# daigo0927/tf-raft

Measured on AMD Instinct MI355X. Metric: image-pairs/sec at 448×512 iters_pred=24; final-iter EPE vs TF ref, higher is better.
Workload: dtype f32; 1 GPU; RAFT forward BASELINE configs[1]: batch 4/GPU 448x512 iters_pred=24 random weights; pairs_per_gpu=4, global_batch=4, parallelism=dp1, collective=none

## Files before the change

tf_raft_amd/csrc/conv_wino4.h:

```cpp
#pragma once
#include "conv_mfma.h"

typedef float f32x2 __attribute__((ext_vector_type(2)));
typedef unsigned int u32x2 __attribute__((ext_vector_type(2)));

#include <type_traits>
#include <utility>

#ifdef RAFT_WINO4_SCALAR
struct alignas(8) w4v2 {
    float x, y;
    __device__ __forceinline__ float operator[](int i) const { return i ? y : x; }
};
__device__ __forceinline__ w4v2 operator+(w4v2 a, w4v2 b) { return {a.x + b.x, a.y + b.y}; }
__device__ __forceinline__ w4v2 operator-(w4v2 a, w4v2 b) { return {a.x - b.x, a.y - b.y}; }
__device__ __forceinline__ w4v2 operator*(float k, w4v2 a) { return {k * a.x, k * a.y}; }
#else
typedef f32x2 w4v2;
#endif

template <class F, int... I>
__device__ __forceinline__ void w4_static_for_impl(F &f, std::integer_sequence<int, I...>) {
    (f(std::integral_constant<int, I>{}), ...);
}
template <int N, class F>
__device__ __forceinline__ void w4_static_for(F &&f) {
    w4_static_for_impl(f, std::make_integer_sequence<int, N>{});
}
#define W4_TAPS(X)                                                                                                       \
    X(0) X(1) X(2) X(3) X(4) X(5) X(6) X(7) X(8) X(9) X(10) X(11) X(12) X(13) X(14) X(15) X(16) X(17) X(18) X(19) X(20) X(21)   \
    X(22) X(23) X(24) X(25) X(26) X(27) X(28) X(29) X(30) X(31) X(32) X(33) X(34) X(35)

#ifndef RAFT_WINO4_PF
#define RAFT_WINO4_PF 7
#endif
#ifdef RAFT_WINO4_NOSB
#define W4_SB()
#else
#define W4_SB() __builtin_amdgcn_sched_barrier(0)
#endif
#ifdef RAFT_WINO4_NOSNOP
#define W4_PAD ""
#else
#define W4_PAD "s_nop 1\n\t"
#endif
#define W4_MFMA4                                                                                                          \
    W4_PAD "v_mfma_f32_16x16x4_f32 %0, %2, %4, %0\n\tv_mfma_f32_16x16x4_f32 %1, %2, %6, %1\n\t"                          \
           "v_mfma_f32_16x16x4_f32 %0, %3, %5, %0\n\tv_mfma_f32_16x16x4_f32 %1, %3, %7, %1"
#ifndef RAFT_WINO4_ATAPS
#define RAFT_WINO4_ATAPS 31
#endif
#ifndef RAFT_WINO4_ABL
#define RAFT_WINO4_ABL 0
#endif

namespace wino4 {
constexpr float PA = 0.625f, PB = 1.5f;
constexpr float A2 = PA * PA, B2 = PB * PB, SS = A2 + B2, PP = A2 * B2, A3 = A2 * PA, B3 = B2 * PB;
constexpr int TW = 64, HWP = TW + 2;
constexpr int RS = 1124;
constexpr int NTHR = 256;
constexpr int PF = RAFT_WINO4_PF, NR = 8;
constexpr int W4_ATAPS = RAFT_WINO4_ATAPS;
#ifndef RAFT_WINO4_LAG
#define RAFT_WINO4_LAG 12
#endif
constexpr int LOAD_SLOT0 = 0, STORE_LAG = RAFT_WINO4_LAG;
static_assert(PF >= 1 && PF < NR, "prefetch distance must fit the fragment ring");
__device__ __forceinline__ constexpr int tap_row(int ph, int row) { return ph == 0 ? 1 + row : (ph == 1 ? 3 + row : 5 * row); }
}

#pragma clang diagnostic push
#pragma clang diagnostic ignored "-Wunused-lambda-capture"
template <int EPI, int KS = 1, int PRE = 0, int STATS = 0>
__global__ void __launch_bounds__(256, 1) conv_wino4_kernel(ConvArgs p) {
    using namespace wino4;
    static_assert(EPI == EPI_LINEAR || EPI == EPI_RELU || EPI == EPI_RES, "winograd F(4x4) kernel: linear / relu / residual epilogues");
    static_assert(KS == 1 || KS == 2, "K split: 1 or 2");
    static_assert((!PRE && !STATS) || KS == 1, "encoder variants: two row blocks per workgroup");
    constexpr int TH = KS == 1 ? 8 : 4, HH = TH + 2, HP = HH * HWP;
    constexpr int A_BUF = HH * RS + 16;
    constexpr int NA = (HP * 4 * KS + NTHR - 1) / NTHR;
    static_assert(LOAD_SLOT0 + NA - 1 + STORE_LAG < 60, "halo writes must precede the chunk's barrier (slot 60)");
    __shared__ __attribute__((aligned(16))) float smem[2 * KS * A_BUF];

    const int tid = threadIdx.x, lane = tid & 63;
    const int w = __builtin_amdgcn_readfirstlane(tid >> 6);
    const int G = lane >> 4, LR = lane & 15;
    const int rb = KS == 1 ? (w & 1) : 0, cbp = KS == 1 ? (w >> 1) : (w & 1), ks = KS == 1 ? 0 : (w >> 1);
    const int tiles_x = (p.W + TW - 1) / TW, tiles_y = (p.H + TH - 1) / TH;
    const int ntn = p.npad / 64;
    const int M = p.B * p.H * p.W;

    int bid = blockIdx.x;
    {
        const int nwg = gridDim.x, xcd = bid & 7, q = nwg >> 3, r = nwg & 7;
        bid = (xcd < r ? xcd * (q + 1) : r * (q + 1) + (xcd - r) * q) + (bid >> 3);
    }
    int mt = bid / ntn, nt = bid - mt * ntn;
#ifdef RAFT_WINO4_XCD
    {
        const int nwg = gridDim.x, xcd = blockIdx.x & 7, idx = blockIdx.x >> 3;
        if ((nwg & 7) == 0 && (ntn & 7) == 0) {
            const int per = ntn >> 3;
            nt = xcd + 8 * (idx % per);
            mt = idx / per;
        } else if ((nwg & 7) == 0 && 8 % ntn == 0) {
            const int g = 8 / ntn;
            nt = xcd % ntn;
            mt = idx * g + xcd / ntn;
        }
    }
#endif
    const int tx0 = mt % tiles_x, ty0 = (mt / tiles_x) % tiles_y, b = mt / (tiles_x * tiles_y);
    const int y0 = ty0 * TH, x0 = tx0 * TW;
    const int n0 = nt * 64;
    const int cin = p.c0 + p.c1;
    const int nch = cin >> 4;
    const int nst = nch / KS;

    const __amdgpu_buffer_rsrc_t rs0 = __builtin_amdgcn_make_buffer_rsrc(
        (void *)p.a0, 0, (int)((((long)M - 1) * p.lda0 + p.c0) * 4), 0x00020000);
    const __amdgpu_buffer_rsrc_t rsw = __builtin_amdgcn_make_buffer_rsrc(
        (void *)p.wp, 0, (int)((long)36 * cin * p.npad * 4), 0x00020000);

    unsigned pixoff[NA];
    int lds_off[NA], pixi[NA];
    unsigned okbits = 0;
#pragma unroll
    for (int i = 0; i < NA; ++i) {
        const int item = tid + NTHR * i;
        const int hq = item >> 2, c4 = item & 3;
        const int s2 = hq / HP, hp = hq - s2 * HP;
        const int hy = hp / HWP, hx = hp - hy * HWP;
        const int yy = y0 - 1 + hy, xx = x0 - 1 + hx;
        const bool ok = (s2 < KS) & ((unsigned)yy < (unsigned)p.H) & ((unsigned)xx < (unsigned)p.W);
        pixi[i] = ok ? (b * p.H + yy) * p.W + xx : -1;
        okbits |= ok ? 1u << i : 0u;
        pixoff[i] = ok ? (unsigned)((pixi[i] * p.lda0 + s2 * 16 + c4 * 4) * 4) : RAFT_OOB;
        lds_off[i] = s2 < KS ? s2 * A_BUF + hy * RS + hx * 16 + (hx >> 2) * 4 + 2 * c4 : HH * RS;
    }
    f32x4 ra[NA];
    f32x2 pre_sc[2], pre_sh[2];
    __amdgpu_buffer_rsrc_t rsn = rs0;
    int soff_n = 0;
    bool on_first = true;
    auto next_source = [&](int st) {
        const int ch = st * 16 * KS;
        const bool first = ch < p.c0, live = st < nst && !(RAFT_WINO4_ABL & 4);
        const float *base = first ? p.a0 : (p.c1 ? p.a1 : p.a0);
        const int ext = first ? (int)((((long)M - 1) * p.lda0 + p.c0) * 4) : (p.c1 ? (int)((((long)M - 1) * p.lda1 + p.c1) * 4) : 0);
        rsn = __builtin_amdgcn_make_buffer_rsrc((void *)base, 0, live ? ext : 0, 0x00020000);
        soff_n = (first ? ch : ch - p.c0) * 4;
        if constexpr (PRE) {
            const int cq = (st < nst ? ch : 0) + (tid & 3) * 4;
            const f32x4 sc = *(const f32x4 *)(p.pre_scale + (long)b * cin + cq), sh = *(const f32x4 *)(p.pre_shift + (long)b * cin + cq);
            pre_sc[0] = f32x2{sc[0], sc[1]};
            pre_sc[1] = f32x2{sc[2], sc[3]};
            pre_sh[0] = f32x2{sh[0], sh[1]};
            pre_sh[1] = f32x2{sh[2], sh[3]};
            return;
        }
        if (on_first && !first) {
            on_first = false;
#pragma unroll
            for (int i = 0; i < NA; ++i)
                pixoff[i] = pixi[i] >= 0 ? (unsigned)((pixi[i] * p.lda1 + (((tid + NTHR * i) >> 2) / HP) * 16 + (tid & 3) * 4) * 4) : RAFT_OOB;
        }
    };
    auto gload_item = [&](int i) {
        ra[i] = __builtin_bit_cast(f32x4, __builtin_amdgcn_raw_buffer_load_b128(rsn, (int)pixoff[i], soff_n, 0));
    };
    auto lstore_item = [&](int i, int buf) {
        float *dst = smem + buf * (KS * A_BUF) + lds_off[i];
        f32x2 lo = f32x2{ra[i][0], ra[i][1]}, hi = f32x2{ra[i][2], ra[i][3]};
        if constexpr (PRE) {
            const bool ok = (okbits >> i) & 1u;
            const f32x2 zero = f32x2{0.f, 0.f};
            lo = __builtin_elementwise_max(__builtin_elementwise_fma(lo, pre_sc[0], pre_sh[0]), zero);
            hi = __builtin_elementwise_max(__builtin_elementwise_fma(hi, pre_sc[1], pre_sh[1]), zero);
            lo = ok ? lo : zero;
            hi = ok ? hi : zero;
        }
        *(f32x2 *)dst = lo;
        *(f32x2 *)(dst + 8) = hi;
    };

    const int a_lane = ks * A_BUF + (4 * rb) * RS + 68 * LR + 2 * G;
    auto rd = [&](int buf, int r, int j, int h) -> w4v2 {
        return *(const w4v2 *)(smem + a_lane + (buf * (KS * A_BUF) + r * RS + 16 * j + 4 * (j >> 2) + 8 * h));
    };
    const unsigned b_lane = (unsigned)(((G * (p.npad >> 5) + (n0 >> 5) + cbp) * 16 + LR) * 16);
    const unsigned qstride = (unsigned)(4 * p.npad) * 8u;
    unsigned wrow = (unsigned)ks * 72u * qstride;
    f32x4 fb[NR];
    auto frag_b = [&](int q, bool skip = false) {
        if (KS == 2 && skip) wrow += 72u * qstride;
        fb[q & (NR - 1)] = __builtin_bit_cast(f32x4, __builtin_amdgcn_raw_buffer_load_b128(rsw, (int)b_lane, (int)wrow, 0));
        wrow += qstride;
        asm volatile("" : "+s"(wrow));
    };

#define X(t) f32x4 accA_##t = f32x4{0.f, 0.f, 0.f, 0.f}, accB_##t = f32x4{0.f, 0.f, 0.f, 0.f};
    W4_TAPS(X)
#undef X
    int acc_end_ = 0;
#define X(t) &accA_##t, &accB_##t,
    auto mma4 = [W4_TAPS(X) & acc_end_](auto tap, float a0, float a1, f32x4 bw) {
#undef X
        constexpr int T = decltype(tap)::value;
#define X(t)                                                                                                                 \
    if constexpr (T == t) {                                                                                                 \
        if constexpr (t < W4_ATAPS)                                                                                         \
            asm volatile(W4_MFMA4 : "+a"(accA_##t), "+a"(accB_##t) : "v"(a0), "v"(a1), "v"(bw[0]), "v"(bw[1]), "v"(bw[2]), "v"(bw[3])); \
        else                                                                                                                \
            asm volatile(W4_MFMA4 : "+v"(accA_##t), "+v"(accB_##t) : "v"(a0), "v"(a1), "v"(bw[0]), "v"(bw[1]), "v"(bw[2]), "v"(bw[3])); \
    }
        W4_TAPS(X)
#undef X
    };
#define X(t) &accA_##t, &accB_##t,
    auto acc_of = [W4_TAPS(X) & acc_end_](auto tile) -> f32x4 {
#undef X
        constexpr int IDX = decltype(tile)::value;
#define X(t)                                       \
    if constexpr (IDX == 2 * t) return accA_##t;   \
    if constexpr (IDX == 2 * t + 1) return accB_##t;
        W4_TAPS(X)
#undef X
    };

    w4v2 R[4][6], W[2][2][6], e0, e5;
    auto s1_pair = [&](int par, int ph, int j) {
        if (RAFT_WINO4_ABL & 2) {
            W[par][0][j] = W[par][1][j] = w4v2{1.f, 1.f};
            return;
        }
        const float c2 = ph == 0 ? B2 : A2, c1 = ph == 0 ? PA : PB;
        const w4v2 t1 = R[3][j] - c2 * R[1][j], t2 = R[2][j] - c2 * R[0][j];
        W[par][0][j] = t1 + c1 * t2;
        W[par][1][j] = t1 - c1 * t2;
    };
    auto s1_edge = [&](int par, int j) {
        if (RAFT_WINO4_ABL & 2) {
            W[par][0][j] = W[par][1][j] = w4v2{1.f, 1.f};
            return;
        }
        W[par][0][j] = (R[3][j] - SS * R[1][j]) + PP * e0;
        W[par][1][j] = (e5 - SS * R[2][j]) + PP * R[0][j];
    };
    w4v2 V[6];
    auto s2_calc = [&](const w4v2 *wr, int tx) {
        if (RAFT_WINO4_ABL & 16) {
            V[tx] = wr[tx];
            return;
        }
        if (tx == 0) {
            V[0] = (wr[4] - SS * wr[2]) + PP * wr[0];
        } else if (tx == 1) {
            const w4v2 t1 = wr[4] - B2 * wr[2], t2 = wr[3] - B2 * wr[1];
            V[1] = t1 + PA * t2;
            V[2] = t1 - PA * t2;
        } else if (tx == 3) {
            const w4v2 t1 = wr[4] - A2 * wr[2], t2 = wr[3] - A2 * wr[1];
            V[3] = t1 + PB * t2;
            V[4] = t1 - PB * t2;
        } else if (tx == 5) {
            V[5] = (wr[5] - SS * wr[3]) + PP * wr[1];
        }
    };

    next_source(0);
#pragma unroll
    for (int i = 0; i < NA; ++i) gload_item(i);
#pragma unroll
    for (int q = 0; q < PF; ++q) frag_b(q);
#pragma unroll
    for (int i = 0; i < NA; ++i) lstore_item(i, 0);
    raft_barrier_lds();
#pragma unroll
    for (int j = 0; j < 6; ++j) {
#pragma unroll
        for (int r = 0; r < 4; ++r) R[r][j] = (RAFT_WINO4_ABL & 2) ? w4v2{1.f, 1.f} : rd(0, r + 1, j, 0);
        s1_pair(0, 0, j);
    }
    s2_calc(W[0][0], 0);

    auto chunk = [&](auto buf_c, int c) {
        constexpr int BUF = decltype(buf_c)::value;
        next_source(c + 1);
        w4_static_for<6>([&](auto inst_c) {
            constexpr int inst = decltype(inst_c)::value;
            constexpr int h = inst / 3, ph = inst % 3, par = inst & 1;
            constexpr int n_h = ph == 2 ? 1 - h : h;
            constexpr int n_buf = (ph == 2 && h == 1) ? 1 - BUF : BUF;
            if (inst == 5) raft_barrier_lds();
            w4_static_for<12>([&](auto u_c) {
                constexpr int u = decltype(u_c)::value;
                constexpr int row = u / 6, tx = u % 6, j = u >> 1;
                constexpr int q = inst * 12 + u;
                constexpr int t = tap_row(ph, row) * 6 + tx;
                if (!(RAFT_WINO4_ABL & 1)) frag_b((q + PF) % 72, q + PF == 72);
                if (!(RAFT_WINO4_ABL & 2)) {
                    if constexpr (ph == 1 && (u & 1) == 0) {
                        e0 = rd(BUF, 0, j, h);
                        e5 = rd(BUF, 5, j, h);
                    }
                    if constexpr (ph == 2 && (u & 1) == 0) {
#pragma unroll
                        for (int r = 0; r < 4; ++r) R[r][j] = rd(n_buf, r + 1, j, n_h);
                    }
                }
                if constexpr ((u & 1) == 1) {
                    if constexpr (ph == 0) s1_pair(par ^ 1, 1, j);
                    if constexpr (ph == 1) s1_edge(par ^ 1, j);
                    if constexpr (ph == 2) s1_pair(par ^ 1, 0, j);
                }
                {
                    constexpr int li = q - LOAD_SLOT0, si = q - LOAD_SLOT0 - STORE_LAG;
                    if constexpr (li >= 0 && li < NA) gload_item(li);
                    if constexpr (si >= 0 && si < NA) lstore_item(si, 1 - BUF);
                }
                W4_SB();
                mma4(std::integral_constant<int, t>{}, V[tx][0], V[tx][1], fb[q & (NR - 1)]);
                W4_SB();
                if constexpr (u < 11) s2_calc(W[par][(u + 1) / 6], (u + 1) % 6);
                if constexpr (u == 11) s2_calc(W[par ^ 1][0], 0);
            });
        });
    };
    for (int st = 0; st < nst; st += 2) {
        chunk(std::integral_constant<int, 0>{}, st);
        chunk(std::integral_constant<int, 1>{}, st + 1);
    }

    asm volatile("s_nop 15\n\ts_nop 15" ::: "memory");
    __builtin_amdgcn_sched_barrier(0);

    constexpr bool HAS_E0 = EPI == EPI_RES;
    const __amdgpu_buffer_rsrc_t ro0 = __builtin_amdgcn_make_buffer_rsrc(
        (void *)p.o0, 0, (int)((((long)M - 1) * p.ldo0 + p.nvalid) * 4), 0x00020000);
    const __amdgpu_buffer_rsrc_t re0 = __builtin_amdgcn_make_buffer_rsrc(
        (void *)(HAS_E0 ? (const void *)p.e0 : (const void *)p.o0), 0,
        HAS_E0 ? (int)((((long)M - 1) * p.lde0 + p.nvalid) * 4) : 0, 0x00020000);
    auto bstore = [](float v, __amdgpu_buffer_rsrc_t r, unsigned voff, int soff) {
        __builtin_amdgcn_raw_buffer_store_b32(__builtin_bit_cast(unsigned, v), r, (int)voff, soff, 0);
    };
    auto bload = [](__amdgpu_buffer_rsrc_t r, unsigned voff, int soff) {
        return __builtin_bit_cast(float, __builtin_amdgcn_raw_buffer_load_b32(r, (int)voff, soff, 0));
    };
    const bool interior = (y0 + TH <= p.H) & (x0 + TW <= p.W);
    int tid_e = threadIdx.x;
    asm volatile("" : "+v"(tid_e));
    const int G_e = (tid_e >> 4) & 3, LR_e = tid_e & 15, rb_e = (tid_e >> 6) & 1, cbp_e = tid_e >> 7;
    const int xb = x0 + 16 * G_e;
    const int ks_e = KS == 1 ? 0 : (tid_e >> 7), cb_e = KS == 1 ? cbp_e : ((tid_e >> 6) & 1), w_e = tid_e >> 6;
    constexpr int NROW = KS == 1 ? 4 : 2;
    unsigned bo[NROW], be[NROW];
    bool rowok[NROW];
#pragma unroll
    for (int i = 0; i < NROW; ++i) {
        const int yy = y0 + (KS == 1 ? 4 * rb_e : 2 * ks_e) + i;
        const unsigned pix0 = (unsigned)((b * p.H + yy) * p.W + xb);
        bo[i] = pix0 * p.ldo0 * 4u;
        be[i] = HAS_E0 ? pix0 * p.lde0 * 4u : 0u;
        rowok[i] = yy < p.H;
    }
    float bias2[2];
    unsigned nofs[2];
    bool nok2[2];
#pragma unroll
    for (int j = 0; j < 2; ++j) {
        const int n = n0 + (cb_e * 2 + j) * 16 + LR_e;
        nok2[j] = n < p.nvalid;
        nofs[j] = (unsigned)n * 4u;
        bias2[j] = p.bias[n];
    }
    float st1[2] = {0.f, 0.f}, st2[2] = {0.f, 0.f};
    auto emit = [&](int j, int i, int rh, const f32x2 *Y) {
        const float bias = bias2[j];
        const unsigned vo = nok2[j] ? bo[i] + nofs[j] : RAFT_OOB, ve = (HAS_E0 && nok2[j]) ? be[i] + nofs[j] : RAFT_OOB;
#pragma unroll
        for (int rr = 0; rr < 2; ++rr) {
            const int r = 2 * rh + rr;
            float xv[4];
            if (HAS_E0) {
#pragma unroll
                for (int jx = 0; jx < 4; ++jx) {
                    const unsigned dead = (interior | (rowok[i] & (xb + 4 * r + jx < p.W))) ? 0u : RAFT_OOB;
                    xv[jx] = bload(re0, ve | dead, (4 * r + jx) * p.lde0 * 4);
                }
            }
#pragma unroll
            for (int jx = 0; jx < 4; ++jx) {
                float v = Y[jx][rr] + bias;
                if (EPI == EPI_RES) {
                    v = fmaxf(xv[jx] + fmaxf(v, 0.f), 0.f);
                } else {
                    if (EPI == EPI_RELU) v = fmaxf(v, 0.f);
                    v *= p.scale;
                }
                if ((RAFT_WINO4_ABL & 8) && v != 12345.678f) continue;
                const unsigned dead = (interior | (rowok[i] & (xb + 4 * r + jx < p.W))) ? 0u : RAFT_OOB;
                if constexpr (STATS) {
                    unsigned dd = dead;
                    asm volatile("" : "+v"(dd));
                    const float vs = __builtin_bit_cast(float, __builtin_bit_cast(unsigned, v) & ~(unsigned)((int)dd >> 31));
                    st1[j] += vs;
                    st2[j] = fmaf(vs, vs, st2[j]);
                }
                bstore(v, ro0, vo | dead, (4 * r + jx) * p.ldo0 * 4);
            }
        }
    };
    f32x2 *xch = (f32x2 *)smem;
    if (KS == 2) raft_barrier_lds();
    w4_static_for<4>([&](auto jr_c) {
        constexpr int j = decltype(jr_c)::value >> 1, rh = decltype(jr_c)::value & 1;
        f32x2 T[4][6], keep[2][4];
        w4_static_for<6>([&](auto tx_c) {
            constexpr int tx = decltype(tx_c)::value;
            auto half = [&](f32x4 a) { return f32x2{a[2 * rh], a[2 * rh + 1]}; };
            const f32x2 m0 = half(acc_of(std::integral_constant<int, 2 * tx + j>{})),
                        m1 = half(acc_of(std::integral_constant<int, 2 * (6 + tx) + j>{})),
                        m2 = half(acc_of(std::integral_constant<int, 2 * (12 + tx) + j>{})),
                        m3 = half(acc_of(std::integral_constant<int, 2 * (18 + tx) + j>{})),
                        m4 = half(acc_of(std::integral_constant<int, 2 * (24 + tx) + j>{})),
                        m5 = half(acc_of(std::integral_constant<int, 2 * (30 + tx) + j>{}));
            const f32x2 sa = m1 + m2, da = m1 - m2, sb = m3 + m4, db = m3 - m4;
            T[0][tx] = m0 + (sa + sb);
            T[1][tx] = PA * da + PB * db;
            T[2][tx] = A2 * sa + B2 * sb;
            T[3][tx] = (A3 * da + B3 * db) + m5;
            __builtin_amdgcn_sched_barrier(0);
        });
#pragma unroll
        for (int i = 0; i < 4; ++i) {
            const f32x2 sa = T[i][1] + T[i][2], da = T[i][1] - T[i][2], sb = T[i][3] + T[i][4], db = T[i][3] - T[i][4];
            f32x2 Y[4];
            Y[0] = T[i][0] + (sa + sb);
            Y[1] = PA * da + PB * db;
            Y[2] = A2 * sa + B2 * sb;
            Y[3] = (A3 * da + B3 * db) + T[i][5];
            if (KS == 1) {
                emit(j, i, rh, Y);
            } else {
                const bool mine = (i >> 1) == ks_e;
#pragma unroll
                for (int jx = 0; jx < 4; ++jx) {
                    if (mine)
                        keep[i & 1][jx] = Y[jx];
                    else
                        xch[(((((j * 2 + rh) * 4 + (w_e ^ 2)) * 2 + (i & 1)) * 4 + jx) << 6) + (tid_e & 63)] = Y[jx];
                }
            }
            __builtin_amdgcn_sched_barrier(0);
        }
        if (KS == 2) {
            raft_barrier_lds();
#pragma unroll
            for (int i2 = 0; i2 < 2; ++i2) {
                f32x2 Y[4];
#pragma unroll
                for (int jx = 0; jx < 4; ++jx)
                    Y[jx] = keep[i2][jx] + xch[(((((j * 2 + rh) * 4 + w_e) * 2 + i2) * 4 + jx) << 6) + (tid_e & 63)];
                emit(j, i2, rh, Y);
            }
        }
    });
    if constexpr (STATS) {
#pragma unroll
        for (int j = 0; j < 2; ++j) {
            float s1 = st1[j], s2 = st2[j];
            s1 += __shfl_xor(s1, 16, 64);
            s2 += __shfl_xor(s2, 16, 64);
            s1 += __shfl_xor(s1, 32, 64);
            s2 += __shfl_xor(s2, 32, 64);
            const int n = n0 + (cb_e * 2 + j) * 16 + LR_e;
            if (G_e == 0) *(float2 *)(p.stats + ((long)(2 * mt + rb_e) * p.npad + n) * 2) = make_float2(s1, s2);
        }
    }
}

#pragma clang diagnostic pop
```

Baseline: 388.2 image-pairs/s.

## Split Winograd tap rows across waves with doubled column tiles and LDS accumulator exchange

Reorganizes the Winograd F(4x4) conv kernel so each wave handles half of the transform tap rows (chosen by th) for all 64 output columns, instead of all taps for a 32-column half. Each A fragment now feeds eight MFMAs across two B fragments, which halves redundant input-transform work per wave. After the main loop, the waves swap their partial accumulators through LDS so each ends up with complete tiles for the epilogue. Prefetch distance, store lag and the AGPR split are retuned to fit the shorter 36-slot loop, at the cost of an extra LDS exchange, two barriers and larger shared memory.

```diff
diff --git a/tf_raft_amd/csrc/conv_wino4.h b/tf_raft_amd/csrc/conv_wino4.h
--- a/tf_raft_amd/csrc/conv_wino4.h
+++ b/tf_raft_amd/csrc/conv_wino4.h
@@ -27,12 +27,10 @@
 __device__ __forceinline__ void w4_static_for(F &&f) {
     w4_static_for_impl(f, std::make_integer_sequence<int, N>{});
 }
-#define W4_TAPS(X)                                                                                                       \
-    X(0) X(1) X(2) X(3) X(4) X(5) X(6) X(7) X(8) X(9) X(10) X(11) X(12) X(13) X(14) X(15) X(16) X(17) X(18) X(19) X(20) X(21)   \
-    X(22) X(23) X(24) X(25) X(26) X(27) X(28) X(29) X(30) X(31) X(32) X(33) X(34) X(35)
+#define W4_LT(X) X(0) X(1) X(2) X(3) X(4) X(5) X(6) X(7) X(8) X(9) X(10) X(11) X(12) X(13) X(14) X(15) X(16) X(17)
 
 #ifndef RAFT_WINO4_PF
-#define RAFT_WINO4_PF 7
+#define RAFT_WINO4_PF 4
 #endif
 #ifdef RAFT_WINO4_NOSB
 #define W4_SB()
@@ -44,11 +42,13 @@
 #else
 #define W4_PAD "s_nop 1\n\t"
 #endif
-#define W4_MFMA4                                                                                                          \
-    W4_PAD "v_mfma_f32_16x16x4_f32 %0, %2, %4, %0\n\tv_mfma_f32_16x16x4_f32 %1, %2, %6, %1\n\t"                          \
-           "v_mfma_f32_16x16x4_f32 %0, %3, %5, %0\n\tv_mfma_f32_16x16x4_f32 %1, %3, %7, %1"
-#ifndef RAFT_WINO4_ATAPS
-#define RAFT_WINO4_ATAPS 31
+#define W4_MFMA8                                                                                                          \
+    W4_PAD "v_mfma_f32_16x16x4_f32 %0, %4, %6, %0\n\tv_mfma_f32_16x16x4_f32 %1, %4, %8, %1\n\t"                          \
+           "v_mfma_f32_16x16x4_f32 %2, %4, %10, %2\n\tv_mfma_f32_16x16x4_f32 %3, %4, %12, %3\n\t"                        \
+           "v_mfma_f32_16x16x4_f32 %0, %5, %7, %0\n\tv_mfma_f32_16x16x4_f32 %1, %5, %9, %1\n\t"                          \
+           "v_mfma_f32_16x16x4_f32 %2, %5, %11, %2\n\tv_mfma_f32_16x16x4_f32 %3, %5, %13, %3"
+#ifndef RAFT_WINO4_ATILES
+#define RAFT_WINO4_ATILES 62
 #endif
 #ifndef RAFT_WINO4_ABL
 #define RAFT_WINO4_ABL 0
@@ -61,13 +61,13 @@
 constexpr int RS = 1124;
 constexpr int NTHR = 256;
 constexpr int PF = RAFT_WINO4_PF, NR = 8;
-constexpr int W4_ATAPS = RAFT_WINO4_ATAPS;
+constexpr int W4_ATILES = RAFT_WINO4_ATILES;
+static_assert(W4_ATILES % 2 == 0 && W4_ATILES <= 64, "AGPR tiles: pairs of column blocks, at most 256 registers");
 #ifndef RAFT_WINO4_LAG
-#define RAFT_WINO4_LAG 12
+#define RAFT_WINO4_LAG 6
 #endif
 constexpr int LOAD_SLOT0 = 0, STORE_LAG = RAFT_WINO4_LAG;
 static_assert(PF >= 1 && PF < NR, "prefetch distance must fit the fragment ring");
-__device__ __forceinline__ constexpr int tap_row(int ph, int row) { return ph == 0 ? 1 + row : (ph == 1 ? 3 + row : 5 * row); }
 }
 
 #pragma clang diagnostic push
@@ -81,13 +81,14 @@
     constexpr int TH = KS == 1 ? 8 : 4, HH = TH + 2, HP = HH * HWP;
     constexpr int A_BUF = HH * RS + 16;
     constexpr int NA = (HP * 4 * KS + NTHR - 1) / NTHR;
-    static_assert(LOAD_SLOT0 + NA - 1 + STORE_LAG < 60, "halo writes must precede the chunk's barrier (slot 60)");
-    __shared__ __attribute__((aligned(16))) float smem[2 * KS * A_BUF];
+    static_assert(LOAD_SLOT0 + NA - 1 + STORE_LAG < 30, "halo writes must precede the chunk's barrier (slot 30)");
+    constexpr int XS = 4 * 36 * 64 * 4;
+    __shared__ __attribute__((aligned(16))) float smem[2 * KS * A_BUF > XS ? 2 * KS * A_BUF : XS];
 
     const int tid = threadIdx.x, lane = tid & 63;
     const int w = __builtin_amdgcn_readfirstlane(tid >> 6);
     const int G = lane >> 4, LR = lane & 15;
-    const int rb = KS == 1 ? (w & 1) : 0, cbp = KS == 1 ? (w >> 1) : (w & 1), ks = KS == 1 ? 0 : (w >> 1);
+    const int rb = KS == 1 ? (w & 1) : 0, th = KS == 1 ? (w >> 1) : (w & 1), ks = KS == 1 ? 0 : (w >> 1);
     const int tiles_x = (p.W + TW - 1) / TW, tiles_y = (p.H + TH - 1) / TH;
     const int ntn = p.npad / 64;
     const int M = p.B * p.H * p.W;
@@ -187,67 +188,84 @@
     };
 
     const int a_lane = ks * A_BUF + (4 * rb) * RS + 68 * LR + 2 * G;
+    const int e_lane = a_lane + th * RS;
     auto rd = [&](int buf, int r, int j, int h) -> w4v2 {
         return *(const w4v2 *)(smem + a_lane + (buf * (KS * A_BUF) + r * RS + 16 * j + 4 * (j >> 2) + 8 * h));
     };
-    const unsigned b_lane = (unsigned)(((G * (p.npad >> 5) + (n0 >> 5) + cbp) * 16 + LR) * 16);
+    auto rd_e = [&](int buf, int r, int j, int h) -> w4v2 {
+        return *(const w4v2 *)(smem + e_lane + (buf * (KS * A_BUF) + r * RS + 16 * j + 4 * (j >> 2) + 8 * h));
+    };
+    const unsigned b_lane = (unsigned)(((G * (p.npad >> 5) + (n0 >> 5)) * 16 + LR) * 16);
     const unsigned qstride = (unsigned)(4 * p.npad) * 8u;
-    unsigned wrow = (unsigned)ks * 72u * qstride;
-    f32x4 fb[NR];
-    auto frag_b = [&](int q, bool skip = false) {
-        if (KS == 2 && skip) wrow += 72u * qstride;
-        fb[q & (NR - 1)] = __builtin_bit_cast(f32x4, __builtin_amdgcn_raw_buffer_load_b128(rsw, (int)b_lane, (int)wrow, 0));
+    const unsigned skip_pe = (unsigned)(12 - 6 * th) * qstride;
+    const unsigned skip_ep = (unsigned)(6 + 6 * th) * qstride;
+    unsigned wrow = ((unsigned)ks * 72u + 12u * (unsigned)th) * qstride;
+    f32x4 fb[NR][2];
+    auto frag_b = [&](int pos, int ring, bool first = false) {
+        if (!first && pos % 18 == 12) wrow += skip_pe;
+        if (!first && pos % 18 == 0) wrow += skip_ep + (KS == 2 && pos == 0 ? 72u * qstride : 0u);
+        fb[ring][0] = __builtin_bit_cast(f32x4, __builtin_amdgcn_raw_buffer_load_b128(rsw, (int)b_lane, (int)wrow, 0));
+        fb[ring][1] = __builtin_bit_cast(f32x4, __builtin_amdgcn_raw_buffer_load_b128(rsw, (int)(b_lane + 256u), (int)wrow, 0));
         wrow += qstride;
         asm volatile("" : "+s"(wrow));
     };
 
-#define X(t) f32x4 accA_##t = f32x4{0.f, 0.f, 0.f, 0.f}, accB_##t = f32x4{0.f, 0.f, 0.f, 0.f};
-    W4_TAPS(X)
+#define X(s) f32x4 acc0_##s = f32x4{0.f, 0.f, 0.f, 0.f}, acc1_##s = f32x4{0.f, 0.f, 0.f, 0.f}, \
+                   acc2_##s = f32x4{0.f, 0.f, 0.f, 0.f}, acc3_##s = f32x4{0.f, 0.f, 0.f, 0.f};
+    W4_LT(X)
 #undef X
     int acc_end_ = 0;
-#define X(t) &accA_##t, &accB_##t,
-    auto mma4 = [W4_TAPS(X) & acc_end_](auto tap, float a0, float a1, f32x4 bw) {
-#undef X
-        constexpr int T = decltype(tap)::value;
-#define X(t)                                                                                                                 \
-    if constexpr (T == t) {                                                                                                 \
-        if constexpr (t < W4_ATAPS)                                                                                         \
-            asm volatile(W4_MFMA4 : "+a"(accA_##t), "+a"(accB_##t) : "v"(a0), "v"(a1), "v"(bw[0]), "v"(bw[1]), "v"(bw[2]), "v"(bw[3])); \
+#define X(s) &acc0_##s, &acc1_##s, &acc2_##s, &acc3_##s,
+    auto mma8 = [W4_LT(X) & acc_end_](auto tap, float a0, float a1, f32x4 b0, f32x4 b1) {
+#undef X
+        constexpr int S = decltype(tap)::value;
+#define W4_OPS(C0, C1, C2, C3, s)                                                                                            \
+    : C0(acc0_##s), C1(acc1_##s), C2(acc2_##s), C3(acc3_##s)                                                                  \
+    : "v"(a0), "v"(a1), "v"(b0[0]), "v"(b0[1]), "v"(b0[2]), "v"(b0[3]), "v"(b1[0]), "v"(b1[1]), "v"(b1[2]), "v"(b1[3])
+#define X(s)                                                                                                                 \
+    if constexpr (S == s) {                                                                                                 \
+        if constexpr (4 * s + 4 <= W4_ATILES)                                                                               \
+            asm volatile(W4_MFMA8 W4_OPS("+a", "+a", "+a", "+a", s));                                                       \
+        else if constexpr (4 * s + 2 <= W4_ATILES)                                                                          \
+            asm volatile(W4_MFMA8 W4_OPS("+a", "+a", "+v", "+v", s));                                                       \
         else                                                                                                                \
-            asm volatile(W4_MFMA4 : "+v"(accA_##t), "+v"(accB_##t) : "v"(a0), "v"(a1), "v"(bw[0]), "v"(bw[1]), "v"(bw[2]), "v"(bw[3])); \
-    }
-        W4_TAPS(X)
-#undef X
-    };
-#define X(t) &accA_##t, &accB_##t,
-    auto acc_of = [W4_TAPS(X) & acc_end_](auto tile) -> f32x4 {
-#undef X
-        constexpr int IDX = decltype(tile)::value;
-#define X(t)                                       \
-    if constexpr (IDX == 2 * t) return accA_##t;   \
-    if constexpr (IDX == 2 * t + 1) return accB_##t;
-        W4_TAPS(X)
-#undef X
-    };
-
-    w4v2 R[4][6], W[2][2][6], e0, e5;
-    auto s1_pair = [&](int par, int ph, int j) {
+            asm volatile(W4_MFMA8 W4_OPS("+v", "+v", "+v", "+v", s));                                                       \
+    }
+        W4_LT(X)
+#undef X
+#undef W4_OPS
+    };
+#define X(s) &acc0_##s, &acc1_##s, &acc2_##s, &acc3_##s,
+    auto acc_of = [W4_LT(X) & acc_end_](auto tile) -> f32x4 {
+#undef X
+        constexpr int IDX = decltype(tile)::value, TAP = IDX >> 1, J = IDX & 1, ROW = TAP / 6, TX = TAP % 6;
+        constexpr int S = (ROW == 0 || ROW == 5 ? 12 : ((ROW - 1) & 1) * 6) + TX, C = (ROW >= 3 ? 2 : 0) + J;
+#define X(s)                                        \
+    if constexpr (S == s && C == 0) return acc0_##s; \
+    if constexpr (S == s && C == 1) return acc1_##s; \
+    if constexpr (S == s && C == 2) return acc2_##s; \
+    if constexpr (S == s && C == 3) return acc3_##s;
+        W4_LT(X)
+#undef X
+    };
+
+    const float c2 = th ? A2 : B2, c1 = th ? PB : PA;
+    w4v2 R[4][6], WP[2][6], WE[6], e_lo, e_mid, e_hi;
+    auto s1_pair = [&](int j) {
         if (RAFT_WINO4_ABL & 2) {
-            W[par][0][j] = W[par][1][j] = w4v2{1.f, 1.f};
+            WP[0][j] = WP[1][j] = w4v2{1.f, 1.f};
             return;
         }
-        const float c2 = ph == 0 ? B2 : A2, c1 = ph == 0 ? PA : PB;
         const w4v2 t1 = R[3][j] - c2 * R[1][j], t2 = R[2][j] - c2 * R[0][j];
-        W[par][0][j] = t1 + c1 * t2;
-        W[par][1][j] = t1 - c1 * t2;
-    };
-    auto s1_edge = [&](int par, int j) {
+        WP[0][j] = t1 + c1 * t2;
+        WP[1][j] = t1 - c1 * t2;
+    };
+    auto s1_edge = [&](int j) {
         if (RAFT_WINO4_ABL & 2) {
-            W[par][0][j] = W[par][1][j] = w4v2{1.f, 1.f};
+            WE[j] = w4v2{1.f, 1.f};
             return;
         }
-        W[par][0][j] = (R[3][j] - SS * R[1][j]) + PP * e0;
-        W[par][1][j] = (e5 - SS * R[2][j]) + PP * R[0][j];
+        WE[j] = (e_hi - SS * e_mid) + PP * e_lo;
     };
     w4v2 V[6];
     auto s2_calc = [&](const w4v2 *wr, int tx) {
@@ -274,7 +292,7 @@
 #pragma unroll
     for (int i = 0; i < NA; ++i) gload_item(i);
 #pragma unroll
-    for (int q = 0; q < PF; ++q) frag_b(q);
+    for (int q = 0; q < PF; ++q) frag_b(q, q, q == 0);
 #pragma unroll
     for (int i = 0; i < NA; ++i) lstore_item(i, 0);
     raft_barrier_lds();
@@ -282,51 +300,47 @@
     for (int j = 0; j < 6; ++j) {
 #pragma unroll
         for (int r = 0; r < 4; ++r) R[r][j] = (RAFT_WINO4_ABL & 2) ? w4v2{1.f, 1.f} : rd(0, r + 1, j, 0);
-        s1_pair(0, 0, j);
-    }
-    s2_calc(W[0][0], 0);
+        if (j < 5) s1_pair(j);
+    }
+    s2_calc(WP[0], 0);
 
     auto chunk = [&](auto buf_c, int c) {
         constexpr int BUF = decltype(buf_c)::value;
         next_source(c + 1);
-        w4_static_for<6>([&](auto inst_c) {
-            constexpr int inst = decltype(inst_c)::value;
-            constexpr int h = inst / 3, ph = inst % 3, par = inst & 1;
-            constexpr int n_h = ph == 2 ? 1 - h : h;
-            constexpr int n_buf = (ph == 2 && h == 1) ? 1 - BUF : BUF;
-            if (inst == 5) raft_barrier_lds();
-            w4_static_for<12>([&](auto u_c) {
-                constexpr int u = decltype(u_c)::value;
-                constexpr int row = u / 6, tx = u % 6, j = u >> 1;
-                constexpr int q = inst * 12 + u;
-                constexpr int t = tap_row(ph, row) * 6 + tx;
-                if (!(RAFT_WINO4_ABL & 1)) frag_b((q + PF) % 72, q + PF == 72);
-                if (!(RAFT_WINO4_ABL & 2)) {
-                    if constexpr (ph == 1 && (u & 1) == 0) {
-                        e0 = rd(BUF, 0, j, h);
-                        e5 = rd(BUF, 5, j, h);
-                    }
-                    if constexpr (ph == 2 && (u & 1) == 0) {
-#pragma unroll
-                        for (int r = 0; r < 4; ++r) R[r][j] = rd(n_buf, r + 1, j, n_h);
-                    }
+        w4_static_for<36>([&](auto i_c) {
+            constexpr int i = decltype(i_c)::value;
+            constexpr int h = i / 18, u = i % 18, g = BUF * 36 + i;
+            constexpr bool PAIR = u < 12;
+            constexpr int tx = PAIR ? u % 6 : u - 12, j = u >> 1;
+            constexpr int n_h = 1 - h, n_buf = h == 1 ? 1 - BUF : BUF;
+            if (i == 30) raft_barrier_lds();
+            if (!(RAFT_WINO4_ABL & 1)) frag_b((i + PF) % 36, (g + PF) % NR);
+            if (!(RAFT_WINO4_ABL & 2)) {
+                if constexpr (PAIR && (u & 1) == 0) {
+                    e_lo = rd_e(BUF, 0, j, h);
+                    e_mid = rd_e(BUF, 2, j, h);
+                    e_hi = rd_e(BUF, 4, j, h);
                 }
-                if constexpr ((u & 1) == 1) {
-                    if constexpr (ph == 0) s1_pair(par ^ 1, 1, j);
-                    if constexpr (ph == 1) s1_edge(par ^ 1, j);
-                    if constexpr (ph == 2) s1_pair(par ^ 1, 0, j);
+                if constexpr (!PAIR) {
+#pragma unroll
+                    for (int r = 0; r < 4; ++r) R[r][tx] = rd(n_buf, r + 1, tx, n_h);
                 }
-                {
-                    constexpr int li = q - LOAD_SLOT0, si = q - LOAD_SLOT0 - STORE_LAG;
-                    if constexpr (li >= 0 && li < NA) gload_item(li);
-                    if constexpr (si >= 0 && si < NA) lstore_item(si, 1 - BUF);
-                }
-                W4_SB();
-                mma4(std::integral_constant<int, t>{}, V[tx][0], V[tx][1], fb[q & (NR - 1)]);
-                W4_SB();
-                if constexpr (u < 11) s2_calc(W[par][(u + 1) / 6], (u + 1) % 6);
-                if constexpr (u == 11) s2_calc(W[par ^ 1][0], 0);
-            });
+            }
+            if constexpr (PAIR && (u & 1) == 1) s1_edge(j);
+            if constexpr (!PAIR && tx >= 1) s1_pair(tx - 1);
+            if constexpr (u == 0) s1_pair(5);
+            {
+                constexpr int li = i - LOAD_SLOT0, si = i - LOAD_SLOT0 - STORE_LAG;
+                if constexpr (li >= 0 && li < NA) gload_item(li);
+                if constexpr (si >= 0 && si < NA) lstore_item(si, 1 - BUF);
+            }
+            W4_SB();
+            mma8(std::integral_constant<int, u>{}, V[tx][0], V[tx][1], fb[g % NR][0], fb[g % NR][1]);
+            W4_SB();
+            if constexpr (PAIR && u < 11) s2_calc(WP[(u + 1) / 6], (u + 1) % 6);
+            if constexpr (u == 11) s2_calc(WE, 0);
+            if constexpr (!PAIR && u < 17) s2_calc(WE, tx + 1);
+            if constexpr (u == 17) s2_calc(WP[0], 0);
         });
     };
     for (int st = 0; st < nst; st += 2) {
@@ -336,6 +350,39 @@
 
     asm volatile("s_nop 15\n\ts_nop 15" ::: "memory");
     __builtin_amdgcn_sched_barrier(0);
+
+    raft_barrier_lds();
+    {
+        const int pw = KS == 1 ? w ^ 2 : w ^ 1;
+        f32x4 *xo = (f32x4 *)smem + pw * (36 * 64) + lane, *xi = (f32x4 *)smem + w * (36 * 64) + lane;
+        if (th) {
+#define X(s)                       \
+    xo[(2 * s) * 64] = acc0_##s; \
+    xo[(2 * s + 1) * 64] = acc1_##s;
+            W4_LT(X)
+#undef X
+        } else {
+#define X(s)                       \
+    xo[(2 * s) * 64] = acc2_##s; \
+    xo[(2 * s + 1) * 64] = acc3_##s;
+            W4_LT(X)
+#undef X
+        }
+        raft_barrier_lds();
+        if (th) {
+#define X(s)                       \
+    acc0_##s = xi[(2 * s) * 64]; \
+    acc1_##s = xi[(2 * s + 1) * 64];
+            W4_LT(X)
+#undef X
+        } else {
+#define X(s)                       \
+    acc2_##s = xi[(2 * s) * 64]; \
+    acc3_##s = xi[(2 * s + 1) * 64];
+            W4_LT(X)
+#undef X
+        }
+    }
 
     constexpr bool HAS_E0 = EPI == EPI_RES;
     const __amdgpu_buffer_rsrc_t ro0 = __builtin_amdgcn_make_buffer_rsrc(
```

Result: faster. 392.4 image-pairs/s, median of 6 (+1.1%).
